# google-deepmind/bsuite

Hardware: NVIDIA H100
Metric: env-steps/sec (higher is better)
Workload: dtype u32 lane state, f64 reward, f32 observation

## Files before the change

### bsuite_b200/_lib.py

```python

import ctypes
import os
import threading

_HERE = os.path.dirname(os.path.abspath(__file__))
LIB_PATH = os.environ.get('BSB_LIBRARY') or os.path.join(_HERE, 'libbsuite_b200.so')

ABI_VERSION = 12
DEVICE_HOST = -1
MAX_INFO = 4
MAX_PACKED_SETTINGS = 64
COMM_ID_BYTES = 128

DEEP_SEA, CATCH, CARTPOLE, CARTPOLE_SWINGUP, MOUNTAIN_CAR, MEMORY_CHAIN, BANDIT, UMBRELLA_CHAIN, \
    DISCOUNTING_CHAIN, MNIST = range(10)
FAMILY_NAMES = ('deep_sea', 'catch', 'cartpole', 'cartpole_swingup', 'mountain_car', 'memory_chain',
                'bandit', 'umbrella_chain', 'discounting_chain', 'mnist')
WRAP_NONE, WRAP_REWARD_NOISE, WRAP_REWARD_SCALE = range(3)
RNG_PHILOX, RNG_MT19937 = range(2)
FLAG_TRACK_EPISODES = 1
FLAG_SAME_STEP_RESET = 2
OBS_FLOAT32, OBS_BFLOAT16, OBS_UINT8 = range(3)
HOST_ORDER_AFTER_STREAM, HOST_PRELAUNCH, HOST_FENCE_CALLER, HOST_NO_WAIT = 1, 2, 4, 8
EPISODE_STAT_FIELDS = ('steps', 'episode', 'total_return', 'episode_len', 'episode_return')


class Config(ctypes.Structure):
  _fields_ = [
      ('family', ctypes.c_int32), ('wrapper', ctypes.c_int32), ('rng_kind', ctypes.c_int32), ('flags', ctypes.c_int32),
      ('size', ctypes.c_int32), ('deterministic', ctypes.c_int32),
      ('rows', ctypes.c_int32), ('columns', ctypes.c_int32),
# ... 12 lines not shown
      ('log_schedule', ctypes.c_void_p), ('log_schedule_len', ctypes.c_int64),
  ]


class ImageDesc(ctypes.Structure):
  _fields_ = [
      ('in_rows', ctypes.c_int32), ('in_cols', ctypes.c_int32), ('out_rows', ctypes.c_int32), ('out_cols', ctypes.c_int32),
      ('channels', ctypes.c_int32), ('row_radius', ctypes.c_int32), ('col_radius', ctypes.c_int32),
      ('reserved0', ctypes.c_int32),
      ('row_index', ctypes.c_void_p), ('row_index_len', ctypes.c_int64),
      ('row_weight', ctypes.c_void_p), ('row_weight_len', ctypes.c_int64),
      ('col_index', ctypes.c_void_p), ('col_index_len', ctypes.c_int64),
      ('col_weight', ctypes.c_void_p), ('col_weight_len', ctypes.c_int64),
      ('row_taps', ctypes.c_void_p), ('row_taps_len', ctypes.c_int64),
      ('col_taps', ctypes.c_void_p), ('col_taps_len', ctypes.c_int64),
  ]


class Outputs(ctypes.Structure):
  _fields_ = [('observation', ctypes.c_void_p), ('reward', ctypes.c_void_p), ('reward_f64', ctypes.c_void_p),
              ('discount', ctypes.c_void_p), ('step_type', ctypes.c_void_p), ('final_observation', ctypes.c_void_p)]


SCORE_MAX_SOURCES = 512
SCORE_QUANTITIES = ('episode', 'total_return', 'total_regret', 'raw_return', 'best_episode', 'total_perfect',
                    'total_bad_episodes')


class ScoreSource(ctypes.Structure):
  _fields_ = [
      ('env', ctypes.c_void_p), ('rows', ctypes.c_void_p), ('counts', ctypes.c_void_p),
      ('n_points', ctypes.c_int32), ('n_columns', ctypes.c_int32), ('lane_stride', ctypes.c_int64),
      ('device', ctypes.c_int32), ('experiment', ctypes.c_int32), ('setting', ctypes.c_int32),
      ('reserved0', ctypes.c_int32), ('first_lane', ctypes.c_int64), ('lanes', ctypes.c_int64),
      ('group_key', ctypes.c_double), ('columns', ctypes.c_int32 * len(SCORE_QUANTITIES)),
      ('reserved1', ctypes.c_int32),
  ]


EXPORTS = {
    'bsb_abi_version': (ctypes.c_int32, []),
    'bsb_last_error': (ctypes.c_char_p, []),
    'bsb_create': (ctypes.c_int32, [ctypes.POINTER(Config), ctypes.c_int64, ctypes.c_int32, ctypes.c_uint64,
                                    ctypes.c_uint64, ctypes.POINTER(ctypes.c_void_p)]),
    'bsb_create_packed': (ctypes.c_int32, [ctypes.POINTER(Config), ctypes.c_int32, ctypes.c_int64, ctypes.c_int32,
                                           ctypes.POINTER(ctypes.c_uint64), ctypes.c_uint64,
                                           ctypes.POINTER(ctypes.c_void_p)]),
    'bsb_packed_layout': (ctypes.c_int32, [ctypes.c_void_p, ctypes.POINTER(ctypes.c_int32), ctypes.POINTER(ctypes.c_int64)]),
    'bsb_destroy': (ctypes.c_int32, [ctypes.c_void_p]),
    'bsb_obs_numel': (ctypes.c_int32, [ctypes.c_void_p, ctypes.POINTER(ctypes.c_int64)]),
    'bsb_obs_shape': (ctypes.c_int32, [ctypes.c_void_p, ctypes.POINTER(ctypes.c_int32), ctypes.POINTER(ctypes.c_int32)]),
    'bsb_num_actions': (ctypes.c_int32, [ctypes.c_void_p, ctypes.POINTER(ctypes.c_int32)]),
    'bsb_batch': (ctypes.c_int32, [ctypes.c_void_p, ctypes.POINTER(ctypes.c_int64)]),
    'bsb_reset': (ctypes.c_int32, [ctypes.c_void_p, ctypes.POINTER(Outputs), ctypes.c_void_p]),
    'bsb_step': (ctypes.c_int32, [ctypes.c_void_p, ctypes.c_void_p, ctypes.POINTER(Outputs), ctypes.c_void_p]),
    'bsb_rollout': (ctypes.c_int32, [ctypes.c_void_p, ctypes.c_int64, ctypes.c_void_p, ctypes.c_uint64,
                                     ctypes.POINTER(Outputs), ctypes.c_void_p, ctypes.c_void_p]),
    'bsb_random_actions': (ctypes.c_int32, [ctypes.c_uint64, ctypes.c_uint64, ctypes.c_int64, ctypes.c_int64,
                                            ctypes.c_int64, ctypes.c_int32, ctypes.c_void_p]),
    'bsb_steps_done': (ctypes.c_int32, [ctypes.c_void_p, ctypes.POINTER(ctypes.c_int64)]),
    'bsb_info_count': (ctypes.c_int32, [ctypes.c_void_p, ctypes.POINTER(ctypes.c_int32)]),
    'bsb_info_name': (ctypes.c_char_p, [ctypes.c_void_p, ctypes.c_int32]),
    'bsb_read_info': (ctypes.c_int32, [ctypes.c_void_p, ctypes.c_int32, ctypes.c_void_p, ctypes.c_void_p]),
    'bsb_read_episode_stats': (ctypes.c_int32, [ctypes.c_void_p, ctypes.c_int32, ctypes.c_void_p, ctypes.c_void_p]),
    'bsb_sum_episode_stats': (ctypes.c_int32, [ctypes.c_void_p, ctypes.c_void_p, ctypes.c_void_p]),
    'bsb_sum_episode_stats_many': (ctypes.c_int32, [ctypes.POINTER(ctypes.c_void_p), ctypes.c_int32, ctypes.c_void_p,
                                                    ctypes.c_void_p]),
    'bsb_log_layout': (ctypes.c_int32, [ctypes.c_void_p, ctypes.POINTER(ctypes.c_int32), ctypes.POINTER(ctypes.c_int32)]),
    'bsb_read_log_rows': (ctypes.c_int32, [ctypes.c_void_p, ctypes.c_void_p, ctypes.c_void_p, ctypes.c_void_p]),
    'bsb_state_bytes': (ctypes.c_int32, [ctypes.c_void_p, ctypes.POINTER(ctypes.c_int64)]),
    'bsb_get_state': (ctypes.c_int32, [ctypes.c_void_p, ctypes.c_void_p, ctypes.c_int64, ctypes.c_void_p]),
    'bsb_set_state': (ctypes.c_int32, [ctypes.c_void_p, ctypes.c_void_p, ctypes.c_int64, ctypes.c_void_p]),
    'bsb_step_host': (ctypes.c_int32, [ctypes.c_void_p, ctypes.c_void_p, ctypes.POINTER(Outputs), ctypes.c_void_p,
                                       ctypes.c_void_p, ctypes.c_uint32]),
    'bsb_host_flush': (ctypes.c_int32, [ctypes.c_void_p]),
    'bsb_host_wait': (ctypes.c_int32, [ctypes.c_void_p]),
    'bsb_host_timing': (ctypes.c_int32, [ctypes.c_void_p, ctypes.c_void_p]),
    'bsb_invalid_actions': (ctypes.c_int32, [ctypes.c_void_p, ctypes.POINTER(ctypes.c_int32)]),
# ... 54 lines not shown
```

### bsuite_b200/csrc/bsb_dispatch.cuh

```cuda
#pragma once
#include <type_traits>
#include <vector>

#include "bsb_env.h"

namespace bsb {

template <class F> struct HostEmit {
  template <class R> static void run(const EnvParams& p, const typename F::Lane& L, R&, float* dst) { F::row(p, L, dst, 1); }
};
template <> struct HostEmit<UmbrellaChain> {
  template <class R> static void run(const EnvParams& p, const UmbrellaChain::Lane& L, R& r, float* dst) { UmbrellaChain::row(p, L, r, dst, 1); }
};
template <> struct HostEmit<DeepSea> {
  template <class R> static void run(const EnvParams& p, const DeepSea::Lane& L, R&, float* dst) {
    for (int e = 0; e < p.obs_numel; ++e) dst[e] = 0.f;
    if (L.hot >= 0) dst[L.hot] = 1.f;
  }
};
template <> struct HostEmit<Catch> {
  template <class R> static void run(const EnvParams& p, const Catch::Lane& L, R&, float* dst) {
    for (int e = 0; e < p.obs_numel; ++e) dst[e] = 0.f;
    dst[L.hot_a] = 1.f; dst[L.hot_b] = 1.f;
  }
// ... 33 lines not shown
    if constexpr (kPacked) { setting_p = p; pack_lane_params(setting_p, lane); }
    const EnvParams& lp = kPacked ? setting_p : p;
    typename F::Lane L;
    R rng, wrng;
    EpisodeStats ep;
    ActionStream action_stream;
    action_stream.open();
    lane_open<F>(lp, lane, L, rng, wrng, ep, a.mode, noise, track);
    if (a.mode == MODE_INIT) F::ctor_draws(lp, L, rng);
    MergedReset<F, R> merged;
    F::init(p, merged.last);
    merged.done = false;
    for (int64_t t = 0; t < a.T; ++t) {
      const int64_t off = t * B + lane;
      int32_t action = 0;
      if (a.mode == MODE_STEP) {
        action = a.actions ? a.actions[off]
                           : action_stream.sample(a.action_seed, lp.lane_offset + (uint64_t)lane, (uint64_t)(a.step0 + t), p.num_actions);
        if (a.actions_out) a.actions_out[off] = action;
      }
      lane_step<F, R, kSameStep>(lp, lane, L, rng, wrng, ep, action, a.mode, noise, track, a.step0 + t, out, off, &merged);
      if constexpr (kSameStep) { if (merged.done && fin) render(lp, merged.last, merged.rng, fin + off * (int64_t)K); }
      render(lp, L, rng, obs + off * (int64_t)K);
    }
    lane_close<F>(lp, lane, L, rng, wrng, ep, noise, track);
  }
}

struct Geometry { int threads = 0; size_t smem = 0; int64_t n_chunks = 0, grid = 0; int extra_blocks = 0; };

template <class F, class O>
int plan_launch(bsb_env* e, LaunchArgs& a, Geometry& g, int extra_threads = 0) {
  const int K = e->p.obs_numel;
  const bool is_onehot = EmitKind<F>::value == EMIT_ONEHOT;
  const bool is_image = EmitKind<F>::value == EMIT_IMAGE;
  const int64_t B = e->p.batch;
  a.emit_bulk = 1;
  a.group_lanes = 1;
  a.work_counter = nullptr;
  a.work_base = 0;
  const size_t elem = sizeof(O);
  a.stage_rows = ((size_t)2 * 32 * (size_t)K * elem <= 14 * 1024) ? 2 : 1;
  if (a.T == 1 && (EmitKind<F>::value == EMIT_ROWS || EmitKind<F>::value == EMIT_TWOHOT)) a.stage_rows = 1;
  a.cta_extra_elems = 0;
  a.bad_action = e->bad_action_dev;
  int chunk = 32;
  if (is_image)
    while (chunk > 8 && (B + chunk - 1) / chunk < 4 * (int64_t)e->num_sms) chunk >>= 1;
  a.chunk_lanes = chunk;
  g.n_chunks = (B + chunk - 1) / chunk;
  int threads = 64;
  bool persistent = false;
  const size_t tile = (size_t)K * elem;
  a.emit_reuse = 0;
  if (is_onehot && a.emit_bulk && g.n_chunks >= 4 * (int64_t)e->num_sms && in_compressed_block(a.obs)) {
    a.emit_bulk = 0;
    a.emit_reuse = a.T == 1 ? 1 : 0;
  }
  if (is_onehot && a.emit_bulk) {
    int m = 1;
    while (m < 16 && (size_t)(2 * m) * tile <= 40 * 1024) m <<= 1;
    if (((size_t)m * tile) % 16 != 0 || (size_t)TILE_STAGES * m * tile > 100 * 1024) {
      a.emit_bulk = 0;
    } else {
      a.group_lanes = m; threads = 32; persistent = true;
    }
  }
  if (is_image && a.emit_bulk) {
    int m = 4;
    while (m > 1 && (size_t)m * tile > 28 * 1024) m >>= 1;
    int mz = 8;
    while (mz > 1 && (size_t)mz * tile > 28 * 1024) mz >>= 1;
    if ((K & 15) != 0 || (size_t)m * tile > 64 * 1024) {
      a.emit_bulk = 0;
    } else {
      a.group_lanes = m; a.stage_rows = 1; threads = 128; a.cta_extra_elems = mz * K; persistent = true;
      if (g.n_chunks < 2 * (int64_t)e->num_sms) threads = 64;
// ... 96 lines not shown
```

### bsuite_b200/csrc/bsb_engine.cu

```cuda
#include <cstdio>
#include <cstdlib>
#include <cstring>
#include <atomic>
#include <chrono>
#if defined(__x86_64__)
#include <immintrin.h>
#endif

#include "bsb_env.h"

using namespace bsb;

namespace bsb {
std::atomic<int64_t> g_launches{0};
namespace { thread_local std::string g_last_error; }
int fail(int code, const std::string& msg) { g_last_error = msg; return code; }
const char* last_error_cstr() { return g_last_error.c_str(); }
}

namespace {

InfoNames info_names(int family) {
  switch (family) {
    case BSB_DEEP_SEA: return {2, {"total_bad_episodes", "denoised_return", nullptr, nullptr}};
    case BSB_CATCH: return {1, {"total_regret", nullptr, nullptr, nullptr}};
    case BSB_CARTPOLE: return {2, {"raw_return", "best_episode", nullptr, nullptr}};
    case BSB_CARTPOLE_SWINGUP: return {3, {"raw_return", "total_upright", "best_episode", nullptr}};
    case BSB_MOUNTAIN_CAR: return {1, {"raw_return", nullptr, nullptr, nullptr}};
    case BSB_MEMORY_CHAIN: return {2, {"total_perfect", "total_regret", nullptr, nullptr}};
    case BSB_BANDIT: return {1, {"total_regret", nullptr, nullptr, nullptr}};
    case BSB_UMBRELLA_CHAIN: return {1, {"total_regret", nullptr, nullptr, nullptr}};
    case BSB_DISCOUNTING_CHAIN: return {0, {nullptr, nullptr, nullptr, nullptr}};
    case BSB_MNIST: return {1, {"total_regret", nullptr, nullptr, nullptr}};
  }
  return {0, {nullptr, nullptr, nullptr, nullptr}};
}

}

namespace {

struct DeviceGuard {
  int prev; bool on;
  explicit DeviceGuard(int dev) : prev(0), on(dev >= 0) { if (on) { cudaGetDevice(&prev); cudaSetDevice(dev); } }
  ~DeviceGuard() { if (on) cudaSetDevice(prev); }
};

int env_alloc(bsb_env* e, void** out, size_t bytes, bool snapshot) {
  if (bytes == 0) { *out = nullptr; return BSB_OK; }
  void* ptr = nullptr;
  if (e->device >= 0) {
    BSB_CUDA(cudaMalloc(&ptr, bytes));
    BSB_CUDA(cudaMemset(ptr, 0, bytes));
  } else {
    ptr = calloc(1, bytes);
    if (!ptr) return fail(BSB_OUT_OF_MEMORY, "calloc failed");
  }
  e->allocs.push_back(ptr);
  if (snapshot) e->state_blocks.push_back(std::make_pair(ptr, bytes));
  *out = ptr;
  return BSB_OK;
}

int env_upload(bsb_env* e, void* dst, const void* src, size_t bytes) {
  if (bytes == 0) return BSB_OK;
  if (e->device >= 0) { BSB_CUDA(cudaMemcpy(dst, src, bytes, cudaMemcpyHostToDevice)); }
  else memcpy(dst, src, bytes);
  return BSB_OK;
}

template <class T> int env_alloc_t(bsb_env* e, T** out, size_t count, bool snapshot) {
  void* ptr = nullptr;
  int rc = env_alloc(e, &ptr, count * sizeof(T), snapshot);
  *out = static_cast<T*>(ptr);
  return rc;
}

int run(bsb_env* e, const LaunchArgs& args, cudaStream_t stream, const TwoPhaseArgs* two_phase = nullptr) {
  DeviceGuard guard(e->device);
  LaunchArgs a = args;
  if (e->device >= 0) {
    cudaStreamCaptureStatus capture = cudaStreamCaptureStatusNone;
    BSB_CUDA(cudaStreamIsCapturing(stream, &capture));
    if (capture != cudaStreamCaptureStatusNone) e->graph_safe = true;
    if (e->graph_safe) a.clock = e->clock;
  }
  return e->variant->run(e, a, stream, two_phase);
}

LaunchArgs make_args(const bsb_env* e, const bsb_outputs* out, const int32_t* actions, int64_t T, int mode) {
  LaunchArgs a;
  memset(&a, 0, sizeof(a));
  a.actions = actions;
  if (out) { a.obs = out->observation; a.reward = out->reward; a.reward_f64 = out->reward_f64; a.discount = out->discount; a.step_type = out->step_type; a.final_obs = out->final_observation; }
  a.T = T; a.step0 = e->steps_done; a.mode = mode;
  const size_t step_bytes = (size_t)e->p.batch * (size_t)e->p.obs_numel * (size_t)e->obs_elem_bytes;
  a.obs_vec_ok = (out && (reinterpret_cast<uintptr_t>(out->observation) % 16 == 0) && (T == 1 || step_bytes % 16 == 0)) ? 1 : 0;
  a.final_vec_ok = (a.final_obs && (reinterpret_cast<uintptr_t>(a.final_obs) % 16 == 0) && (T == 1 || step_bytes % 16 == 0)) ? 1 : 0;
  return a;
}

template <class F> struct FamilyId;
#define BSB_FAMILY_ID(F, id) template <> struct FamilyId<F> { static const int value = id; };
BSB_FAMILY_ID(DeepSea, BSB_DEEP_SEA) BSB_FAMILY_ID(Catch, BSB_CATCH) BSB_FAMILY_ID(Cartpole, BSB_CARTPOLE)
BSB_FAMILY_ID(CartpoleSwingup, BSB_CARTPOLE_SWINGUP) BSB_FAMILY_ID(MountainCar, BSB_MOUNTAIN_CAR)
BSB_FAMILY_ID(MemoryChain, BSB_MEMORY_CHAIN) BSB_FAMILY_ID(Bandit, BSB_BANDIT) BSB_FAMILY_ID(UmbrellaChain, BSB_UMBRELLA_CHAIN)
BSB_FAMILY_ID(DiscountingChain, BSB_DISCOUNTING_CHAIN) BSB_FAMILY_ID(Mnist, BSB_MNIST)
// ... 525 lines not shown

static int check_final_observation(const bsb_env* env, const bsb_outputs* out) {
  if (out->final_observation && !env->same_step)
    return fail(BSB_INVALID_ARGUMENT, "final_observation needs a handle created with BSB_FLAG_SAME_STEP_RESET");
  return BSB_OK;
}

int32_t bsb_reset(bsb_env* env, const bsb_outputs* out, void* stream) {
  if (!env || !out || !out->observation) return fail(BSB_INVALID_ARGUMENT, "bsb_reset needs outputs with an observation buffer");
  { int crc = check_final_observation(env, out); if (crc != BSB_OK) return crc; }
  { int frc = drain_host_steps(env); if (frc != BSB_OK) return frc; }
  LaunchArgs a = make_args(env, out, nullptr, 1, MODE_RESET);
  int rc = run(env, a, static_cast<cudaStream_t>(stream));
  if (rc == BSB_OK) advance_steps(env, 1);
  return rc;
}

int32_t bsb_step(bsb_env* env, const int32_t* actions, const bsb_outputs* out, void* stream) {
  if (!env || !actions || !out || !out->observation) return fail(BSB_INVALID_ARGUMENT, "bsb_step needs actions and outputs with an observation buffer");
  { int crc = check_final_observation(env, out); if (crc != BSB_OK) return crc; }
  { int frc = drain_host_steps(env); if (frc != BSB_OK) return frc; }
  if (env->device < 0) { int vrc = check_host_actions(env, actions, env->p.batch); if (vrc != BSB_OK) return vrc; }
  LaunchArgs a = make_args(env, out, actions, 1, MODE_STEP);
  int rc = run(env, a, static_cast<cudaStream_t>(stream));
  if (rc == BSB_OK) advance_steps(env, 1);
  return rc;
}

int32_t bsb_rollout(bsb_env* env, int64_t num_steps, const int32_t* actions, uint64_t action_seed,
                    const bsb_outputs* out, int32_t* actions_out, void* stream) {
  if (!env || !out || !out->observation) return fail(BSB_INVALID_ARGUMENT, "bsb_rollout needs outputs with an observation buffer");
  if (num_steps <= 0) return fail(BSB_INVALID_ARGUMENT, "num_steps must be positive");
  { int crc = check_final_observation(env, out); if (crc != BSB_OK) return crc; }
  { int frc = drain_host_steps(env); if (frc != BSB_OK) return frc; }
  if (env->device < 0 && actions) { int vrc = check_host_actions(env, actions, num_steps * env->p.batch); if (vrc != BSB_OK) return vrc; }
  LaunchArgs a = make_args(env, out, actions, num_steps, MODE_STEP);
  a.action_seed = action_seed; a.actions_out = actions_out;
  int rc = run(env, a, static_cast<cudaStream_t>(stream));
  if (rc == BSB_OK) advance_steps(env, num_steps);
  return rc;
}

int32_t bsb_random_actions(uint64_t action_seed, uint64_t lane_offset, int64_t batch, int64_t first_step,
                           int64_t num_steps, int32_t num_actions, int32_t* out) {
  if (!out || batch <= 0 || num_steps <= 0 || num_actions <= 0) return fail(BSB_INVALID_ARGUMENT, "bad arguments");
  for (int64_t t = 0; t < num_steps; ++t)
// ... 329 lines not shown
```

### bsuite_b200/csrc/bsb_kernels.cuh

```cuda
#pragma once
#include "bsb_families.cuh"

namespace bsb {

struct MailFields {
  float* reward; double* reward_f64; float* discount; int32_t* step_type;
};

struct LaunchArgs {
  const int32_t* actions;
  int32_t* actions_out;
  float* obs;
  float* reward;
  double* reward_f64;
  float* discount;
  int32_t* step_type;
  int64_t T;
  int64_t step0;
  uint64_t action_seed;
  int32_t mode;
  int32_t obs_vec_ok;
  int32_t emit_bulk;
  int32_t emit_reuse;
  int32_t use_pdl;
  int32_t group_lanes;
  int32_t final_vec_ok;
  unsigned long long* work_counter;
  unsigned long long work_base;
  unsigned long long* clock;
  int32_t chunk_lanes;
  int32_t stage_rows;
  int32_t cta_extra_elems;
  struct HostMailbox* mailbox;
  struct DeviceMail* mail;
  unsigned long long ticket;
  int32_t timing;
  float* final_obs;
  int32_t* bad_action;
};

struct TwoPhaseArgs {
  int32_t copiers;
  MailFields stage;
};

struct HostMailbox {
  volatile unsigned long long done;     unsigned long long pad[7];
  volatile unsigned long long stamp[8];
};
struct DeviceMail {
  unsigned long long last_exit;
  unsigned long long finished;
  volatile unsigned long long phase1;
  unsigned long long copied;
};

enum { MODE_STEP = 0, MODE_RESET = 1, MODE_INIT = 2 };

enum { NEXT_STEP = 0, SAME_STEP = 1, PACKED = 2 };
template <class Family, class O, int kMode> struct Variant {
  typedef Family Fam;
// ... 341 lines not shown
    const uint4* slot = ring + (s % REUSE_STAGES) * REUSE_WORDS;
    if (!blind) cp_async_wait<REUSE_STAGES - 1>();
    unsigned differing = 0;
#pragma unroll 2
    for (int u = 0; u < REUSE_WORDS / 32 && u * 32 < KV - q0; ++u) {
      const int q = u * 32 + tid;
      const bool in = q0 + q < KV;
      const uint4 v = onehot_word<O>(h, q0 + q);
      const bool differs = in && (blind || bits_differ(slot[q], v));
      const unsigned mask = __ballot_sync(0xffffffffu, differs);
      differing += __popc(mask);
      const unsigned block = (unsigned)((1ull << REUSE_STORE_WORDS) - 1ull) << (tid & ~(REUSE_STORE_WORDS - 1));
      if (in && (mask & block) != 0u) __stcs(dst + q, v);
    }
    if (!blind) {
      blind = differing > 2u;
      if (!blind) reuse_load(ring, obs_t, warp_base, n_lanes, K, s + REUSE_STAGES);
    }
  }
  cp_async_wait<0>();
}

template <class O>
__device__ __forceinline__ void emit_twohot_vec(O* obs_t, int64_t warp_base, int n_lanes, int K, int hot_a, int hot_b, bool vec) {
  const int tid = threadIdx.x & 31;
  const int total = n_lanes * K;
  O* dst = obs_t + warp_base * (int64_t)K;
  constexpr int S = Vec16<O>::shift;
  if (vec && sizeof(O) != 4 && (total & ((1 << S) - 1)) == 0) {
    const int totalV = total >> S;
    for (int q0 = 0; q0 < totalV; q0 += 32) {
      const int q = q0 + tid;
      const int e0 = (q < totalV ? q : 0) << S;
      int j = e0 / K, c = e0 - j * K;
      uint32_t w[4] = {0u, 0u, 0u, 0u};
#pragma unroll
      for (int k = 0; k < (1 << S); ++k) {
        const int jj = j < 32 ? j : 31;
        const int a = __shfl_sync(0xffffffffu, hot_a, jj);
        const int b = __shfl_sync(0xffffffffu, hot_b, jj);
        if (c == a || c == b) w[(k * (int)sizeof(O)) >> 2] |= one_bits<O>() << (((k * (int)sizeof(O)) & 3) * 8);
        if (++c >= K) { c = 0; ++j; }
      }
      if (q < totalV) __stcs(reinterpret_cast<uint4*>(dst) + q, make_uint4(w[0], w[1], w[2], w[3]));
    }
  } else if (vec && (total & ((1 << S) - 1)) == 0) {
// ... 238 lines not shown
  const int K = p.obs_numel;
  bool bulk = a.emit_bulk && vec;
  if (kEmit == EMIT_ROWS) bulk = bulk && K >= 3 && ((n_lanes * K) & V1) == 0;
  if (kEmit == EMIT_TWOHOT) bulk = bulk && ((n_lanes * K) & V1) == 0;
  if (kEmit == EMIT_ONEHOT) bulk = bulk && ((K & V1) == 0 || ((n_lanes % a.group_lanes) == 0 && ((a.group_lanes * K) & V1) == 0));
  if (kEmit == EMIT_IMAGE) bulk = bulk && (K & 3) == 0;
  return bulk;
}
template <class O>
__device__ __forceinline__ bool reuse_chunk(const LaunchArgs& a, bool vec, int K) {
  return a.emit_reuse && vec && (K & ((1 << Vec16<O>::shift) - 1)) == 0;
}

template <class F, class O, class R>
__device__ __forceinline__ void emit_obs(const EnvParams& p, const LaunchArgs& a, WarpStage<O>& ws, const typename F::Lane& L,
                                         R& rng, O* obs_t, int64_t warp_base, int n_lanes, int64_t lane, bool active,
                                         bool bulk, bool vec, bool reuse = true) {
  constexpr int kEmit = EmitKind<F>::value;
  constexpr int V1 = (1 << Vec16<O>::shift) - 1;
  const int tid = threadIdx.x & 31;
  const int K = p.obs_numel;
  if (kEmit == EMIT_ONEHOT) {
    const int hot = Descriptor<F>::a(L);
    if (bulk) {
      const int m = a.group_lanes;
      for (int g0 = 0; g0 < n_lanes; g0 += m) {
        const int in_group = (n_lanes - g0) < m ? (n_lanes - g0) : m;
        const int s = (int)(ws.emitted & 1u);
        O* group = ws.stage + (size_t)s * m * K;
        if (tid == 0) bulk_wait_read<TILE_STAGES - 1>();
        __syncwarp();
        if (s == 0) { if (ws.tile_poked0 >= 0) { group[ws.tile_poked0] = obs_cast<O>(0.f); ws.tile_poked0 = -1; } }
        else        { if (ws.tile_poked1 >= 0) { group[ws.tile_poked1] = obs_cast<O>(0.f); ws.tile_poked1 = -1; } }
        __syncwarp();
        if (tid >= g0 && tid < g0 + in_group && hot >= 0) {
          const int cell = (tid - g0) * K + hot;
          group[cell] = obs_cast<O>(1.f);
          if (s == 0) ws.tile_poked0 = cell; else ws.tile_poked1 = cell;
        }
        fence_proxy_async_smem();
        __syncwarp();
        if (tid == 0) {
          O* tile_dst = obs_t + (warp_base + g0) * (int64_t)K;
          const uint32_t tile_bytes = (uint32_t)in_group * (uint32_t)K * (uint32_t)sizeof(O);
          bulk_store_obs(tile_dst, group, tile_bytes);
          bulk_commit();
        }
        ++ws.emitted;
      }
    } else if (reuse && reuse_chunk<O>(a, vec, K)) {
      emit_onehot_reuse(reinterpret_cast<uint4*>(ws.stage), obs_t, warp_base, n_lanes, K, hot);
    } else {
      emit_onehot_vec(obs_t, warp_base, n_lanes, K, hot, vec && (K & V1) == 0);
    }
  } else if (kEmit == EMIT_TWOHOT) {
    const int hot_a = Descriptor<F>::a(L), hot_b = Descriptor<F>::b(L);
    if (bulk) {
      const int buf = (int)(ws.emitted & ws.row_mask);
      O* boards = ws.stage + (size_t)buf * 32 * K;
      if (tid == 0) { if (ws.row_mask) bulk_wait_read<1>(); else bulk_wait_read<0>(); }
      __syncwarp();
      O* mine = boards + tid * K;
      const int old_a = buf ? ws.poked_a1 : ws.poked_a0, old_b = buf ? ws.poked_b1 : ws.poked_b0;
      if (old_a >= 0) mine[old_a] = obs_cast<O>(0.f);
      if (old_b >= 0) mine[old_b] = obs_cast<O>(0.f);
      int new_a = -1, new_b = -1;
      if (active) { mine[hot_a] = obs_cast<O>(1.f); mine[hot_b] = obs_cast<O>(1.f); new_a = hot_a; new_b = hot_b; }
      if (buf) { ws.poked_a1 = new_a; ws.poked_b1 = new_b; } else { ws.poked_a0 = new_a; ws.poked_b0 = new_b; }
      fence_proxy_async_smem();
      __syncwarp();
      if (tid == 0) { bulk_store_obs(obs_t + warp_base * (int64_t)K, boards, (uint32_t)n_lanes * (uint32_t)K * (uint32_t)sizeof(O)); bulk_commit(); }
      ++ws.emitted;
    } else {
      emit_twohot_vec(obs_t, warp_base, n_lanes, K, hot_a, hot_b, vec);
    }
  } else if (kEmit == EMIT_IMAGE) {
    const int image = Descriptor<F>::a(L);
// ... 322 lines not shown
```

### bsuite_b200/environment.py

```python

import ctypes
from typing import Any, Dict, Optional

import numpy as np

from bsuite_b200 import _lib
from bsuite_b200 import dm_env
from bsuite_b200 import obs_memory
from bsuite_b200.experiments import EnvSpec

specs = dm_env.specs

_INT_INFO = frozenset(['total_bad_episodes', 'total_perfect'])
_MASK64 = (1 << 64) - 1


def _fresh_seed() -> int:
  return int(np.random.SeedSequence().generate_state(1, dtype=np.uint32)[0])


def _resolve_device(device) -> int:
  import torch
  if device is None:
    device = 'cuda'
# ... 69 lines not shown
    self.lib = _lib.load()
    built = [_make_config(spec, _lib.RNG_PHILOX, flags, log_schedule) for spec in specs]
    configs = (_lib.Config * len(built))(*[cfg for cfg, _ in built])
    seed_array = (ctypes.c_uint64 * len(seeds))(*[int(s) & _MASK64 for s in seeds])
    ptr = ctypes.c_void_p()
    _lib.check(self.lib.bsb_create_packed(configs, len(built), int(lanes_per_setting), device_ordinal, seed_array,
                                          lane_offset & _MASK64, ctypes.byref(ptr)))
    del built
    self.ptr = ptr
    return self

  def close(self):
    if self.ptr is not None and self.ptr.value:
      self.lib.bsb_destroy(self.ptr)
      self.ptr = None

  def __del__(self):
    try:
      self.close()
    except Exception:
      pass


class StepBuffers:

  def __init__(self, observation, reward, discount, step_type, actions=None, final_observation=None):
    self.observation = observation
    self.reward = reward
    self.discount = discount
    self.step_type = step_type
    self.actions = actions
    self.final_observation = final_observation
    self._outputs = None
    self._bound = None
    self._timestep = None

  def as_outputs(self) -> _lib.Outputs:
    if self._outputs is None:
      self._outputs = self._build_outputs()
    return self._outputs

  def bind(self, obs_dtype) -> _lib.Outputs:
    if self._bound is not obs_dtype:
      for name in ('observation', 'final_observation'):
        tensor = getattr(self, name)
        if tensor is not None and tensor.dtype != obs_dtype:
          raise ValueError(f'out.{name} is {tensor.dtype}, but this environment writes {obs_dtype} '
                           'observations (obs_dtype)')
      self._bound = obs_dtype
    return self.as_outputs()

  def _build_outputs(self) -> _lib.Outputs:
    import torch
    out = _lib.Outputs()
    if self.observation is not None:
      out.observation = self.observation.data_ptr()
    if self.reward is not None:
      if self.reward.dtype == torch.float64:
        out.reward_f64 = self.reward.data_ptr()
      else:
        out.reward = self.reward.data_ptr()
    if self.discount is not None:
      out.discount = self.discount.data_ptr()
    if self.step_type is not None:
      out.step_type = self.step_type.data_ptr()
    if self.final_observation is not None:
      out.final_observation = self.final_observation.data_ptr()
    return out

  def timestep(self) -> 'dm_env.TimeStep':
    if self._timestep is None:
      self._timestep = dm_env.TimeStep(step_type=self.step_type, reward=self.reward, discount=self.discount,
                                       observation=self.observation)
    return self._timestep


class GraphedSteps:

  def __init__(self, env, graph, actions, buffers):
    self.env = env
    self.graph = graph
    self.actions = actions
    self.buffers = buffers
    self.timestep = buffers.timestep()

  def replay(self):
    self.graph.replay()
    return self.timestep


class BatchedEnvironment:

  def __init__(self, spec: EnvSpec, batch: int, device='cuda', seed: Optional[int] = None,
               rng: str = 'philox', lane_offset: int = 0, track_episodes: bool = False,
               reward_dtype='float32', record_rows: bool = False, obs_dtype='float32', autoreset: str = 'next_step',
               _pack=None):
    import torch
    self._torch = torch
    self._spec = spec
    self._batch = int(batch)
    self._ordinal = _resolve_device(device)
    self._device = torch.device('cpu') if self._ordinal < 0 else torch.device('cuda', self._ordinal)
    if rng not in ('philox', 'mt19937'):
      raise ValueError(f'rng must be "philox" or "mt19937", got {rng!r}')
    self._rng_kind = _lib.RNG_PHILOX if rng == 'philox' else _lib.RNG_MT19937
    seed = seed if seed is not None else spec.seed
    self._seed = _fresh_seed() if seed is None else int(seed)
    if self._rng_kind == _lib.RNG_MT19937 and not 0 <= self._seed < 2**32:
      raise ValueError('Seed must be between 0 and 2**32 - 1')
# ... 56 lines not shown
      lo, hi = self._spec.obs_bounds
      return specs.BoundedArray(shape=self._spec.obs_shape, dtype=np.float32, name=self._spec.obs_spec_name,
                                minimum=lo, maximum=hi)
    return specs.Array(shape=self._spec.obs_shape, dtype=np.float32, name=self._spec.obs_spec_name)

  def action_spec(self):
    return specs.DiscreteArray(self._spec.num_actions, dtype=self._spec.action_dtype, name='action')

  def make_buffers(self, num_steps: Optional[int] = None, with_actions: bool = False,
                   final_observation: bool = False) -> StepBuffers:
    torch = self._torch
    if final_observation and self._autoreset != 'same_step':
      raise ValueError("final_observation needs autoreset='same_step'")
    lead = (self._batch,) if num_steps is None else (int(num_steps), self._batch)
    kw = dict(device=self._device)
    obs_shape = lead + tuple(self._spec.obs_shape)
    obs_args = (obs_shape, self._obs_dtype, self._device, self._spec.family)
    return StepBuffers(
        observation=obs_memory.empty(*obs_args),
        reward=torch.empty(lead, dtype=self._reward_dtype, **kw),
        discount=torch.empty(lead, dtype=torch.float32, **kw),
        step_type=torch.empty(lead, dtype=torch.int32, **kw),
        actions=torch.empty(lead, dtype=torch.int32, **kw) if with_actions else None,
        final_observation=obs_memory.empty(*obs_args, zero=True) if final_observation else None)

  def _stream(self):
    if self._ordinal < 0:
      return None
    raw = getattr(self._torch._C, '_cuda_getCurrentRawStream', None)
    if raw is not None:
      return raw(self._ordinal)
    return self._torch.cuda.current_stream(self._device).cuda_stream

  def _device_actions(self, actions, shape):
    torch = self._torch
    if not isinstance(actions, torch.Tensor):
      actions = torch.as_tensor(np.asarray(actions))
    if tuple(actions.shape) != tuple(shape):
      raise ValueError(f'actions must have shape {tuple(shape)}, got {tuple(actions.shape)}')
    if actions.dtype != torch.int32 or actions.device != self._device or not actions.is_contiguous():
      actions = actions.to(device=self._device, dtype=torch.int32, non_blocking=True).contiguous()
    return actions

  def reset(self, out: Optional[StepBuffers] = None):
    out = out or self.make_buffers()
    outputs = out.bind(self._obs_dtype)
    self._async_work = True
    _lib.check(self._lib.bsb_reset(self._handle.ptr, ctypes.byref(outputs), self._stream()))
    return out.timestep()

  def step(self, actions, out: Optional[StepBuffers] = None):
    torch = self._torch
    if not (type(actions) is torch.Tensor and actions.dtype is torch.int32 and actions.dim() == 1
            and actions.shape[0] == self._batch and actions.is_contiguous()
            and (actions.device == self._device
                 or (self._ordinal >= 0 and actions.device.type == 'cpu' and actions.is_pinned()))):
      actions = self._device_actions(actions, (self._batch,))
    if out is None:
      out = self.make_buffers()
    self._async_work = True
    outputs = out._outputs if out._bound is self._obs_dtype else out.bind(self._obs_dtype)
    status = self._lib.bsb_step(self._handle.ptr, actions.data_ptr(), ctypes.byref(outputs), self._stream())
    if status:
      _lib.check(status)
    return out.timestep()

  def make_mixed_buffers(self) -> StepBuffers:
    torch = self._torch
    if self._ordinal < 0:
      return self.make_buffers()
    host = self.make_host_buffers()
    return StepBuffers(observation=obs_memory.empty((self._batch,) + tuple(self._spec.obs_shape), self._obs_dtype,
                                                    self._device, self._spec.family),
                       reward=host.reward, discount=host.discount, step_type=host.step_type)

  def make_host_buffers(self, with_observation: bool = False) -> StepBuffers:
    torch = self._torch
    pin = self._ordinal >= 0
    B = self._batch
    if self._reward_dtype == torch.float32:
      block = torch.empty(3 * B, dtype=torch.float32, pin_memory=pin)
      reward, discount, step_type = block[:B], block[B:2 * B], block[2 * B:].view(torch.int32)
    else:
      reward = torch.empty(B, dtype=torch.float64, pin_memory=pin)
      discount = torch.empty(B, dtype=torch.float32, pin_memory=pin)
      step_type = torch.empty(B, dtype=torch.int32, pin_memory=pin)
    observation = (torch.empty((B,) + tuple(self._spec.obs_shape), dtype=self._obs_dtype, pin_memory=pin)
                   if with_observation else None)
    return StepBuffers(observation=observation, reward=reward, discount=discount, step_type=step_type)

  def step_host(self, actions, host: StepBuffers, out: Optional[StepBuffers] = None, prelaunch: bool = False,
                wait: bool = True):
    torch = self._torch
    if not (type(actions) is torch.Tensor and actions.dtype is torch.int32 and actions.device.type == 'cpu'
            and actions.dim() == 1 and actions.shape[0] == self._batch and actions.is_contiguous()):
      if not isinstance(actions, torch.Tensor):
        actions = torch.as_tensor(np.asarray(actions))
      if actions.device.type != 'cpu' or actions.dtype != torch.int32 or tuple(actions.shape) != (self._batch,):
        raise ValueError('step_host takes a CPU int32 tensor of shape [batch]')
      actions = actions.contiguous()
    if out is None:
      out = self.make_buffers()
    if host.final_observation is not None:
      raise ValueError('step_host does not deliver final observations')
    houts = host._outputs if host._bound is self._obs_dtype else host.bind(self._obs_dtype)
    if out._bound is not self._obs_dtype:
      out.bind(self._obs_dtype)
    dev_obs = None if self._ordinal < 0 else out.observation.data_ptr()
    if self._ordinal < 0:
      houts = _lib.Outputs.from_buffer_copy(houts)
      houts.observation = out.observation.data_ptr()
    flags = (_lib.HOST_PRELAUNCH if prelaunch else 0) | (0 if wait else _lib.HOST_NO_WAIT)
    stream = None
    if self._ordinal >= 0:
      flags |= _lib.HOST_FENCE_CALLER
      stream = self._stream()
      if self._async_work:
        flags |= _lib.HOST_ORDER_AFTER_STREAM
        self._async_work = False
    status = self._lib.bsb_step_host(self._handle.ptr, actions.data_ptr(), ctypes.byref(houts), dev_obs, stream, flags)
    if status:
      _lib.check(status)
    if self._ordinal < 0 and host.observation is not None:
      host.observation.copy_(out.observation)
    return host.timestep(), out.observation

  def host_wait(self):
    status = self._lib.bsb_host_wait(self._handle.ptr)
    if status:
      _lib.check(status)

  def host_flush(self):
    _lib.check(self._lib.bsb_host_flush(self._handle.ptr))

  def invalid_actions_seen(self) -> bool:
    if self._ordinal >= 0:
      self._torch.cuda.current_stream(self._device).synchronize()
    seen = ctypes.c_int32()
    _lib.check(self._lib.bsb_invalid_actions(self._handle.ptr, ctypes.byref(seen)))
    return bool(seen.value)

  def rollout(self, num_steps: int, actions=None, action_seed: int = 0, out: Optional[StepBuffers] = None):
    num_steps = int(num_steps)
    out = out or self.make_buffers(num_steps, with_actions=actions is None)
    act_ptr = None
    if actions is not None:
      actions = self._device_actions(actions, (num_steps, self._batch))
      act_ptr = ctypes.c_void_p(actions.data_ptr())
    outputs = out.bind(self._obs_dtype)
    act_out = ctypes.c_void_p(out.actions.data_ptr()) if out.actions is not None else None
    self._async_work = True
    _lib.check(self._lib.bsb_rollout(self._handle.ptr, num_steps, act_ptr, int(action_seed) & _MASK64,
                                     ctypes.byref(outputs), act_out, self._stream()))
    return out.timestep()

  def capture(self, num_steps: int = 1, sample_actions: bool = False, fused: bool = False,
              action_seed: int = 0, final_observation: bool = False) -> GraphedSteps:
    torch = self._torch
    if self._ordinal < 0:
      raise RuntimeError('CUDA graphs need a CUDA environment')
    T = int(num_steps)
    buffers = self.make_buffers(T, with_actions=sample_actions, final_observation=final_observation)
    actions = None if sample_actions else torch.zeros((T, self._batch), dtype=torch.int32, device=self._device)
    slices = [StepBuffers(buffers.observation[t:t + 1], buffers.reward[t:t + 1], buffers.discount[t:t + 1],
                          buffers.step_type[t:t + 1], None if buffers.actions is None else buffers.actions[t:t + 1],
                          None if buffers.final_observation is None else buffers.final_observation[t:t + 1])
              for t in range(T)]

    def record():
      if fused:
        self.rollout(T, actions=actions, action_seed=action_seed, out=buffers)
      else:
        for t in range(T):
          self.rollout(1, actions=None if actions is None else actions[t:t + 1], action_seed=action_seed, out=slices[t])
# ... 150 lines not shown
      import torch
      device_t = torch.device('cuda', self._ordinal)
      self._dev = StepBuffers(
          observation=torch.empty(numel, dtype=torch.float32, device=device_t),
          reward=torch.empty(1, dtype=torch.float64, device=device_t),
          discount=torch.empty(1, dtype=torch.float32, device=device_t),
          step_type=torch.empty(1, dtype=torch.int32, device=device_t))

  def _timestep(self):
    code = self._step_type_c.value
    observation = self._obs_view.copy()
    if code == 0:
      return dm_env.TimeStep(self._step_types[0], None, None, observation)
    return dm_env.TimeStep(self._step_types[code], self._reward_c.value, self._discount_c.value, observation)

  def reset(self):
    if self._ordinal < 0:
      _lib.check(self._lib.bsb_reset(self._handle.ptr, ctypes.byref(self._outputs), None))
    else:
      import torch
      outputs = self._dev.as_outputs()
      stream = ctypes.c_void_p(torch.cuda.current_stream(self._dev.observation.device).cuda_stream)
      self._reset_stream, self._host_flags = stream, _lib.HOST_ORDER_AFTER_STREAM
      _lib.check(self._lib.bsb_reset(self._handle.ptr, ctypes.byref(outputs), stream))
      self._obs[:] = self._dev.observation.cpu().numpy()
      self._reward[:] = self._dev.reward.cpu().numpy()
      self._discount[:] = self._dev.discount.cpu().numpy()
      self._step_type[:] = self._dev.step_type.cpu().numpy()
    return self._timestep()

  def step(self, action):
    action = int(action)
    if not 0 <= action < self._spec.num_actions:
      raise ValueError(f'action {action} is outside the action_spec: DiscreteArray(num_values={self._spec.num_actions})')
    self._action_c.value = action
    if self._ordinal < 0:
      status = self._lib.bsb_step(self._handle.ptr, self._action_ptr, self._outputs_ref, None)
    else:
      status = self._lib.bsb_step_host(self._handle.ptr, self._action_ptr, self._outputs_ref, None, self._reset_stream,
                                       self._host_flags)
      self._host_flags = 0
    if status:
      _lib.check(status)
    return self._timestep()

  def observation_spec(self):
# ... 31 lines not shown
```

### bsuite_b200/suite.py

```python

from typing import Dict, List, Optional, Sequence

from bsuite_b200 import distributed
from bsuite_b200 import registry
from bsuite_b200 import sweep


def one_per_experiment(setting: int = 0) -> List[str]:
  return [ids[min(setting, len(ids) - 1)] for ids in sweep.BY_EXPERIMENT.values()]


_STATE_BYTES = {0: 8, 1: 8, 2: 80, 3: 80, 4: 48}


def algorithmic_bytes_per_lane_step(env) -> int:
  numel = 1
  for d in env.obs_shape:
    numel *= d
  return 4 * numel + 16 + _STATE_BYTES.get(env.family, 16)


class GraphedSweep:

  def __init__(self, graph, timesteps):
    self.graph, self.timesteps = graph, timesteps

  def replay(self):
    self.graph.replay()
    return self.timesteps


class SweepBatch:

  def __init__(self, bsuite_ids: Optional[Sequence[str]] = None, lanes: int = 4096, device='cuda', seed: int = 0,
               rank: int = 0, world: int = 1, track_episodes: bool = True, ring: int = 1,
               autoreset: str = 'next_step', record_rows: bool = False):
    import torch
    self._torch = torch
    self.bsuite_ids = list(bsuite_ids) if bsuite_ids is not None else one_per_experiment()
    first, count = distributed.shard_range(lanes, rank, world)
    self.lanes, self.local_lanes, self.lane_offset = lanes, count, first
    self.envs = {
        bsuite_id: registry.load_from_id(bsuite_id, batch=count, device=device, seed=seed, lane_offset=first,
                                         track_episodes=track_episodes, autoreset=autoreset,
                                         record_rows=record_rows)
        for bsuite_id in self.bsuite_ids
    }
    self._device = next(iter(self.envs.values())).device
    self._cuda = self._device.type == 'cuda'
    self._streams = {k: torch.cuda.Stream(device=self._device) for k in self.envs} if self._cuda else {}
# ... 92 lines not shown
```

### include/bsuite_b200.h

```cpp
#ifndef BSUITE_B200_H_
#define BSUITE_B200_H_

#include <stddef.h>
#include <stdint.h>

#ifdef __cplusplus
extern "C" {
#endif

#define BSB_ABI_VERSION 12
#define BSB_DEVICE_HOST (-1)
#define BSB_MAX_INFO 4
#define BSB_MAX_PACKED_SETTINGS 64

typedef enum bsb_status {
  BSB_OK = 0,
  BSB_INVALID_ARGUMENT = 1,
  BSB_UNSUPPORTED = 2,
  BSB_CUDA_ERROR = 3,
  BSB_OUT_OF_MEMORY = 4,
  BSB_INTERNAL = 5
} bsb_status;

typedef enum bsb_step_type { BSB_FIRST = 0, BSB_MID = 1, BSB_LAST = 2 } bsb_step_type;

typedef enum bsb_family {
  BSB_DEEP_SEA = 0,
  BSB_CATCH = 1,
  BSB_CARTPOLE = 2,
  BSB_CARTPOLE_SWINGUP = 3,
  BSB_MOUNTAIN_CAR = 4,
  BSB_MEMORY_CHAIN = 5,
  BSB_BANDIT = 6,
// ... 73 lines not shown

int32_t bsb_create(const bsb_config* config, int64_t batch, int32_t device,
                   uint64_t seed, uint64_t lane_offset, bsb_env** out);

int32_t bsb_create_packed(const bsb_config* configs, int32_t n_settings,
                          int64_t lanes_per_setting, int32_t device,
                          const uint64_t* seeds, uint64_t lane_offset,
                          bsb_env** out);

int32_t bsb_packed_layout(const bsb_env* env, int32_t* n_settings,
                          int64_t* lanes_per_setting);

int32_t bsb_destroy(bsb_env* env);

int32_t bsb_obs_numel(const bsb_env* env, int64_t* numel);
int32_t bsb_obs_shape(const bsb_env* env, int32_t* rows, int32_t* cols);
int32_t bsb_num_actions(const bsb_env* env, int32_t* num_actions);
int32_t bsb_batch(const bsb_env* env, int64_t* batch);

int32_t bsb_reset(bsb_env* env, const bsb_outputs* out, void* stream);

int32_t bsb_step(bsb_env* env, const int32_t* actions, const bsb_outputs* out,
                 void* stream);

int32_t bsb_rollout(bsb_env* env, int64_t num_steps, const int32_t* actions,
                    uint64_t action_seed, const bsb_outputs* out,
                    int32_t* actions_out, void* stream);

int32_t bsb_random_actions(uint64_t action_seed, uint64_t lane_offset,
                           int64_t batch, int64_t first_step, int64_t num_steps,
                           int32_t num_actions, int32_t* out);

int32_t bsb_steps_done(const bsb_env* env, int64_t* steps);

int32_t bsb_info_count(const bsb_env* env, int32_t* count);
const char* bsb_info_name(const bsb_env* env, int32_t index);
int32_t bsb_read_info(bsb_env* env, int32_t index, double* dst, void* stream);

int32_t bsb_read_episode_stats(bsb_env* env, int32_t field, double* dst,
                               void* stream);


int32_t bsb_sum_episode_stats(bsb_env* env, double* dst5, void* stream);

int32_t bsb_sum_episode_stats_many(bsb_env* const* envs, int32_t count,
                                   double* dst, void* stream);
// ... 117 lines not shown
```

Measured before the change: 926.7 million.

## Write only changed cache lines of one-hot DeepSea observations on tracked steps

Adds a tracked step entry point that records each lane's previous hot cell on device. When the Python layer can prove the observation buffer was not modified since the engine last wrote it, the kernel rewrites only the cache lines holding the old and new hot cells instead of the whole one-hot tile. This cuts per-step observation write bandwidth for DeepSea. In exchange it needs a host-side version and write-count bookkeeping to decide trust, and it disables the delta path under graph capture. It also skips redundant cudaSetDevice calls in DeviceGuard.

Result: faster. 1.796 billion, median of 6 (+93.8%).

```diff
diff --git a/bsuite_b200/_lib.py b/bsuite_b200/_lib.py
--- a/bsuite_b200/_lib.py
+++ b/bsuite_b200/_lib.py
@@ -6,7 +6,7 @@
 _HERE = os.path.dirname(os.path.abspath(__file__))
 LIB_PATH = os.environ.get('BSB_LIBRARY') or os.path.join(_HERE, 'libbsuite_b200.so')
 
-ABI_VERSION = 12
+ABI_VERSION = 13
 DEVICE_HOST = -1
 MAX_INFO = 4
 MAX_PACKED_SETTINGS = 64
@@ -65,6 +65,10 @@
               ('discount', ctypes.c_void_p), ('step_type', ctypes.c_void_p), ('final_observation', ctypes.c_void_p)]
 
 
+class ObsTrack(ctypes.Structure):
+  _fields_ = [('hot', ctypes.c_void_p), ('trusted', ctypes.c_int32), ('reserved', ctypes.c_int32)]
+
+
 SCORE_MAX_SOURCES = 512
 SCORE_QUANTITIES = ('episode', 'total_return', 'total_regret', 'raw_return', 'best_episode', 'total_perfect',
                     'total_bad_episodes')
@@ -97,6 +101,8 @@
     'bsb_batch': (ctypes.c_int32, [ctypes.c_void_p, ctypes.POINTER(ctypes.c_int64)]),
     'bsb_reset': (ctypes.c_int32, [ctypes.c_void_p, ctypes.POINTER(Outputs), ctypes.c_void_p]),
     'bsb_step': (ctypes.c_int32, [ctypes.c_void_p, ctypes.c_void_p, ctypes.POINTER(Outputs), ctypes.c_void_p]),
+    'bsb_step_tracked': (ctypes.c_int32, [ctypes.c_void_p, ctypes.c_void_p, ctypes.POINTER(Outputs),
+                                          ctypes.POINTER(ObsTrack), ctypes.c_void_p]),
     'bsb_rollout': (ctypes.c_int32, [ctypes.c_void_p, ctypes.c_int64, ctypes.c_void_p, ctypes.c_uint64,
                                      ctypes.POINTER(Outputs), ctypes.c_void_p, ctypes.c_void_p]),
     'bsb_random_actions': (ctypes.c_int32, [ctypes.c_uint64, ctypes.c_uint64, ctypes.c_int64, ctypes.c_int64,
diff --git a/bsuite_b200/csrc/bsb_dispatch.cuh b/bsuite_b200/csrc/bsb_dispatch.cuh
--- a/bsuite_b200/csrc/bsb_dispatch.cuh
+++ b/bsuite_b200/csrc/bsb_dispatch.cuh
@@ -79,6 +79,7 @@
       lane_step<F, R, kSameStep>(lp, lane, L, rng, wrng, ep, action, a.mode, noise, track, a.step0 + t, out, off, &merged);
       if constexpr (kSameStep) { if (merged.done && fin) render(lp, merged.last, merged.rng, fin + off * (int64_t)K); }
       render(lp, L, rng, obs + off * (int64_t)K);
+      if constexpr (EmitKind<F>::value == EMIT_ONEHOT) { if (a.hot_rec && a.T == 1) a.hot_rec[lane] = L.hot; }
     }
     lane_close<F>(lp, lane, L, rng, wrng, ep, noise, track);
   }
@@ -110,6 +111,9 @@
   bool persistent = false;
   const size_t tile = (size_t)K * elem;
   a.emit_reuse = 0;
+  if (!is_onehot || a.T != 1) a.hot_rec = nullptr;
+  a.emit_delta = (a.emit_delta && a.hot_rec && a.obs_vec_ok && tile % 16 == 0) ? 1 : 0;
+  if (a.emit_delta) a.emit_bulk = 0;
   if (is_onehot && a.emit_bulk && g.n_chunks >= 4 * (int64_t)e->num_sms && in_compressed_block(a.obs)) {
     a.emit_bulk = 0;
     a.emit_reuse = a.T == 1 ? 1 : 0;
diff --git a/bsuite_b200/csrc/bsb_engine.cu b/bsuite_b200/csrc/bsb_engine.cu
--- a/bsuite_b200/csrc/bsb_engine.cu
+++ b/bsuite_b200/csrc/bsb_engine.cu
@@ -42,7 +42,9 @@
 
 struct DeviceGuard {
   int prev; bool on;
-  explicit DeviceGuard(int dev) : prev(0), on(dev >= 0) { if (on) { cudaGetDevice(&prev); cudaSetDevice(dev); } }
+  explicit DeviceGuard(int dev) : prev(0), on(dev >= 0) {
+    if (on) { cudaGetDevice(&prev); on = prev != dev; if (on) cudaSetDevice(dev); }
+  }
   ~DeviceGuard() { if (on) cudaSetDevice(prev); }
 };
 
@@ -82,7 +84,10 @@
   if (e->device >= 0) {
     cudaStreamCaptureStatus capture = cudaStreamCaptureStatusNone;
     BSB_CUDA(cudaStreamIsCapturing(stream, &capture));
-    if (capture != cudaStreamCaptureStatusNone) e->graph_safe = true;
+    if (capture != cudaStreamCaptureStatusNone) {
+      e->graph_safe = true;
+      a.emit_delta = 0;
+    }
     if (e->graph_safe) a.clock = e->clock;
   }
   return e->variant->run(e, a, stream, two_phase);
@@ -654,6 +659,23 @@
   { int frc = drain_host_steps(env); if (frc != BSB_OK) return frc; }
   if (env->device < 0) { int vrc = check_host_actions(env, actions, env->p.batch); if (vrc != BSB_OK) return vrc; }
   LaunchArgs a = make_args(env, out, actions, 1, MODE_STEP);
+  int rc = run(env, a, static_cast<cudaStream_t>(stream));
+  if (rc == BSB_OK) advance_steps(env, 1);
+  return rc;
+}
+
+int32_t bsb_step_tracked(bsb_env* env, const int32_t* actions, const bsb_outputs* out, const bsb_obs_track* track,
+                         void* stream) {
+  if (!track) return bsb_step(env, actions, out, stream);
+  if (!env || !actions || !out || !out->observation) return fail(BSB_INVALID_ARGUMENT, "bsb_step_tracked needs actions and outputs with an observation buffer");
+  if (!track->hot) return fail(BSB_INVALID_ARGUMENT, "bsb_step_tracked needs a hot-cell record (bsb_obs_track.hot)");
+  if (track->reserved != 0) return fail(BSB_INVALID_ARGUMENT, "bsb_obs_track.reserved must be 0");
+  { int crc = check_final_observation(env, out); if (crc != BSB_OK) return crc; }
+  { int frc = drain_host_steps(env); if (frc != BSB_OK) return frc; }
+  if (env->device < 0) { int vrc = check_host_actions(env, actions, env->p.batch); if (vrc != BSB_OK) return vrc; }
+  LaunchArgs a = make_args(env, out, actions, 1, MODE_STEP);
+  a.hot_rec = track->hot;
+  a.emit_delta = (track->trusted != 0 && env->device >= 0) ? 1 : 0;
   int rc = run(env, a, static_cast<cudaStream_t>(stream));
   if (rc == BSB_OK) advance_steps(env, 1);
   return rc;
diff --git a/bsuite_b200/csrc/bsb_kernels.cuh b/bsuite_b200/csrc/bsb_kernels.cuh
--- a/bsuite_b200/csrc/bsb_kernels.cuh
+++ b/bsuite_b200/csrc/bsb_kernels.cuh
@@ -37,6 +37,8 @@
   int32_t timing;
   float* final_obs;
   int32_t* bad_action;
+  int32_t* hot_rec;
+  int32_t emit_delta;
 };
 
 struct TwoPhaseArgs {
@@ -424,6 +426,28 @@
 }
 
 template <class O>
+__device__ __forceinline__ void emit_onehot_delta(O* obs_t, int64_t warp_base, int n_lanes, int K, int hot, int old) {
+  constexpr int S = Vec16<O>::shift;
+  constexpr int LINE_WORDS = 8;
+  const int tid = threadIdx.x & 31;
+  const int KV = K >> S;
+  const int half = tid >> 4, which = (tid >> 3) & 1, w = tid & (LINE_WORDS - 1);
+  for (int j0 = 0; j0 < n_lanes; j0 += 2) {
+    const int j = j0 + half;
+    const int src = j < 32 ? j : 31;
+    const int hn = __shfl_sync(0xffffffffu, hot, src), ho = __shfl_sync(0xffffffffu, old, src);
+    if (j >= n_lanes) continue;
+    uint4* const tile = reinterpret_cast<uint4*>(obs_t + (warp_base + j) * (int64_t)K);
+    const int64_t lead = (int64_t)((reinterpret_cast<uintptr_t>(tile) & 127u) >> 4);
+    auto line_of = [&](int h) { return (int)((lead + (h >> S)) / LINE_WORDS); };
+    const int h = which ? hn : ho;
+    if (h < 0 || (!which && hn >= 0 && line_of(ho) == line_of(hn))) continue;
+    const int q = line_of(h) * LINE_WORDS + w - (int)lead;
+    if (q >= 0 && q < KV) __stcs(tile + q, onehot_word<O>(hn, q));
+  }
+}
+
+template <class O>
 __device__ __forceinline__ void emit_twohot_vec(O* obs_t, int64_t warp_base, int n_lanes, int K, int hot_a, int hot_b, bool vec) {
   const int tid = threadIdx.x & 31;
   const int total = n_lanes * K;
@@ -708,7 +732,9 @@
   const int K = p.obs_numel;
   if (kEmit == EMIT_ONEHOT) {
     const int hot = Descriptor<F>::a(L);
-    if (bulk) {
+    if (reuse && a.emit_delta) {
+      emit_onehot_delta(obs_t, warp_base, n_lanes, K, hot, active ? a.hot_rec[lane] : -1);
+    } else if (bulk) {
       const int m = a.group_lanes;
       for (int g0 = 0; g0 < n_lanes; g0 += m) {
         const int in_group = (n_lanes - g0) < m ? (n_lanes - g0) : m;
@@ -739,6 +765,7 @@
     } else {
       emit_onehot_vec(obs_t, warp_base, n_lanes, K, hot, vec && (K & V1) == 0);
     }
+    if (reuse && a.hot_rec && active) a.hot_rec[lane] = hot;
   } else if (kEmit == EMIT_TWOHOT) {
     const int hot_a = Descriptor<F>::a(L), hot_b = Descriptor<F>::b(L);
     if (bulk) {
diff --git a/bsuite_b200/environment.py b/bsuite_b200/environment.py
--- a/bsuite_b200/environment.py
+++ b/bsuite_b200/environment.py
@@ -115,22 +115,69 @@
       pass
 
 
+_ENGINE_WRITES: Dict[int, int] = {}
+
+OBSERVATION_WRITERS = (
+    'environment.BatchedEnvironment.step',
+    'environment.BatchedEnvironment.reset',
+    'environment.BatchedEnvironment.rollout',
+    'environment.BatchedEnvironment.step_host',
+    'environment.GraphedSteps.replay',
+    'environment.DmEnvAdapter.reset',
+    'suite.GraphedSweep.replay',
+)
+
+_ONE_HOT_FAMILIES = frozenset([_lib.DEEP_SEA])
+
+
+def storage_key(tensor) -> int:
+  return tensor.untyped_storage().data_ptr()
+
+
+def engine_writes(tensor) -> int:
+  return _ENGINE_WRITES.get(storage_key(tensor), 0)
+
+
+def _note_writes(keys):
+  for key in keys:
+    _ENGINE_WRITES[key] = _ENGINE_WRITES.get(key, 0) + 1
+
+
+def note_engine_write(*tensors):
+  _note_writes([storage_key(t) for t in tensors if t is not None])
+
+
 class StepBuffers:
 
-  def __init__(self, observation, reward, discount, step_type, actions=None, final_observation=None):
+  def __init__(self, observation, reward, discount, step_type, actions=None, final_observation=None, hot=None):
     self.observation = observation
     self.reward = reward
     self.discount = discount
     self.step_type = step_type
     self.actions = actions
     self.final_observation = final_observation
+    self.hot = hot
     self._outputs = None
     self._bound = None
     self._timestep = None
+    self._write_keys = ()
+    self._track = None
+    self._track_ref = None
+    self._outputs_ref = None
+    self._trust = None
+
+  def forget(self):
+    self._trust = None
 
   def as_outputs(self) -> _lib.Outputs:
     if self._outputs is None:
       self._outputs = self._build_outputs()
+      self._write_keys = tuple(storage_key(t) for t in (self.observation, self.final_observation) if t is not None)
+      if self.hot is not None and self.observation is not None and not self.observation.is_inference():
+        self._track = _lib.ObsTrack()
+        self._track.hot = self.hot.data_ptr()
+        self._track_ref = ctypes.byref(self._track)
+        self._outputs_ref = ctypes.byref(self._outputs)
     return self._outputs
 
   def bind(self, obs_dtype) -> _lib.Outputs:
@@ -176,8 +223,10 @@
     self.actions = actions
     self.buffers = buffers
     self.timestep = buffers.timestep()
+    self._write_keys = [storage_key(t) for t in (buffers.observation, buffers.final_observation) if t is not None]
 
   def replay(self):
+    _note_writes(self._write_keys)
     self.graph.replay()
     return self.timestep
 
@@ -280,7 +329,13 @@
         discount=torch.empty(lead, dtype=torch.float32, **kw),
         step_type=torch.empty(lead, dtype=torch.int32, **kw),
         actions=torch.empty(lead, dtype=torch.int32, **kw) if with_actions else None,
-        final_observation=obs_memory.empty(*obs_args, zero=True) if final_observation else None)
+        final_observation=obs_memory.empty(*obs_args, zero=True) if final_observation else None,
+        hot=self._hot_record() if num_steps is None else None)
+
+  def _hot_record(self):
+    if self._ordinal < 0 or self._spec.family not in _ONE_HOT_FAMILIES:
+      return None
+    return self._torch.full((self._batch,), -1, dtype=self._torch.int32, device=self._device)
 
   def _stream(self):
     if self._ordinal < 0:
@@ -304,21 +359,35 @@
     out = out or self.make_buffers()
     outputs = out.bind(self._obs_dtype)
     self._async_work = True
+    _note_writes(out._write_keys)
     _lib.check(self._lib.bsb_reset(self._handle.ptr, ctypes.byref(outputs), self._stream()))
     return out.timestep()
 
   def step(self, actions, out: Optional[StepBuffers] = None):
     torch = self._torch
     if not (type(actions) is torch.Tensor and actions.dtype is torch.int32 and actions.dim() == 1
-            and actions.shape[0] == self._batch and actions.is_contiguous()
-            and (actions.device == self._device
+            and actions.size(0) == self._batch and actions.is_contiguous()
+            and (actions.get_device() == self._ordinal
                  or (self._ordinal >= 0 and actions.device.type == 'cpu' and actions.is_pinned()))):
       actions = self._device_actions(actions, (self._batch,))
     if out is None:
       out = self.make_buffers()
     self._async_work = True
     outputs = out._outputs if out._bound is self._obs_dtype else out.bind(self._obs_dtype)
-    status = self._lib.bsb_step(self._handle.ptr, actions.data_ptr(), ctypes.byref(outputs), self._stream())
+    track = out._track
+    if track is None:
+      _note_writes(out._write_keys)
+      status = self._lib.bsb_step(self._handle.ptr, actions.data_ptr(), ctypes.byref(outputs), self._stream())
+    else:
+      key = out._write_keys[0]
+      seen = (out.observation._version, _ENGINE_WRITES.get(key, 0))
+      track.trusted = out._trust == seen
+      if len(out._write_keys) > 1:
+        _note_writes(out._write_keys[1:])
+      _ENGINE_WRITES[key] = seen[1] + 1
+      status = self._lib.bsb_step_tracked(self._handle.ptr, actions.data_ptr(), out._outputs_ref, out._track_ref,
+                                          self._stream())
+      out._trust = None if status else (seen[0], seen[1] + 1)
     if status:
       _lib.check(status)
     return out.timestep()
@@ -330,7 +399,7 @@
     host = self.make_host_buffers()
     return StepBuffers(observation=obs_memory.empty((self._batch,) + tuple(self._spec.obs_shape), self._obs_dtype,
                                                     self._device, self._spec.family),
-                       reward=host.reward, discount=host.discount, step_type=host.step_type)
+                       reward=host.reward, discount=host.discount, step_type=host.step_type, hot=self._hot_record())
 
   def make_host_buffers(self, with_observation: bool = False) -> StepBuffers:
     torch = self._torch
@@ -364,6 +433,8 @@
     houts = host._outputs if host._bound is self._obs_dtype else host.bind(self._obs_dtype)
     if out._bound is not self._obs_dtype:
       out.bind(self._obs_dtype)
+    _note_writes(out._write_keys)
+    _note_writes(host._write_keys)
     dev_obs = None if self._ordinal < 0 else out.observation.data_ptr()
     if self._ordinal < 0:
       houts = _lib.Outputs.from_buffer_copy(houts)
@@ -408,6 +479,7 @@
     outputs = out.bind(self._obs_dtype)
     act_out = ctypes.c_void_p(out.actions.data_ptr()) if out.actions is not None else None
     self._async_work = True
+    _note_writes(out._write_keys)
     _lib.check(self._lib.bsb_rollout(self._handle.ptr, num_steps, act_ptr, int(action_seed) & _MASK64,
                                      ctypes.byref(outputs), act_out, self._stream()))
     return out.timestep()
@@ -604,6 +676,7 @@
       outputs = self._dev.as_outputs()
       stream = ctypes.c_void_p(torch.cuda.current_stream(self._dev.observation.device).cuda_stream)
       self._reset_stream, self._host_flags = stream, _lib.HOST_ORDER_AFTER_STREAM
+      _note_writes(self._dev._write_keys)
       _lib.check(self._lib.bsb_reset(self._handle.ptr, ctypes.byref(outputs), stream))
       self._obs[:] = self._dev.observation.cpu().numpy()
       self._reward[:] = self._dev.reward.cpu().numpy()
diff --git a/bsuite_b200/suite.py b/bsuite_b200/suite.py
--- a/bsuite_b200/suite.py
+++ b/bsuite_b200/suite.py
@@ -2,6 +2,7 @@
 from typing import Dict, List, Optional, Sequence
 
 from bsuite_b200 import distributed
+from bsuite_b200 import environment
 from bsuite_b200 import registry
 from bsuite_b200 import sweep
 
@@ -24,8 +25,11 @@
 
   def __init__(self, graph, timesteps):
     self.graph, self.timesteps = graph, timesteps
+    steps = timesteps if isinstance(timesteps, list) else [timesteps]
+    self._observations = [ts.observation for lock_step in steps for ts in lock_step.values()]
 
   def replay(self):
+    environment.note_engine_write(*self._observations)
     self.graph.replay()
     return self.timesteps
 
diff --git a/include/bsuite_b200.h b/include/bsuite_b200.h
--- a/include/bsuite_b200.h
+++ b/include/bsuite_b200.h
@@ -8,7 +8,7 @@
 extern "C" {
 #endif
 
-#define BSB_ABI_VERSION 12
+#define BSB_ABI_VERSION 13
 #define BSB_DEVICE_HOST (-1)
 #define BSB_MAX_INFO 4
 #define BSB_MAX_PACKED_SETTINGS 64
@@ -128,6 +128,16 @@
 
 int32_t bsb_step(bsb_env* env, const int32_t* actions, const bsb_outputs* out,
                  void* stream);
+
+typedef struct bsb_obs_track {
+  int32_t* hot;
+  int32_t trusted;
+  int32_t reserved;
+} bsb_obs_track;
+
+int32_t bsb_step_tracked(bsb_env* env, const int32_t* actions,
+                         const bsb_outputs* out, const bsb_obs_track* track,
+                         void* stream);
 
 int32_t bsb_rollout(bsb_env* env, int64_t num_steps, const int32_t* actions,
                     uint64_t action_seed, const bsb_outputs* out,
```
